# mezis/blurrily

Measured on AMD Instinct MI355X. Metric: find() queries/sec (batched), Geonames-scale haystack, higher is better.
Workload: dtype u32; 1 GPU; configs[2]: synthetic Geonames-scale haystack, 1M batched needles; haystack_strings=8423769, haystack_entries=117301316, needles_per_gpu=1000000, limit=10, index_replicated=False, parallelism=query-shard x1

## Files before the change

### blurrily_amd/csrc/find_kernels.h

```cpp
#pragma once
#include <hip/hip_runtime.h>

#include <cstddef>
#include <cstdint>

#include "../../include/blurrily_storage.h"
#include "device_index.h"

namespace blurrily {

struct TokeniseArgs {
  const char*     packed;
  const uint64_t* offsets;
  uint32_t        n;
  const uint32_t* code_total;
  uint16_t*       qcodes;
  uint32_t*       q_ntri;
  uint32_t*       q_nb;
  uint32_t*       big_list;
  uint32_t*       big_count;
  uint32_t*       mid_list;
  uint32_t*       mid_count;
  const uint32_t* start_win;
  uint32_t*       q_start;
  uint32_t        max_len;
};

struct FindArgs {
  const uint2*    slice_se;
  const uint16_t* ent;
  const uint32_t* ref_of_rank;
  const uint32_t* weight_of_rank;
  uint32_t        n_refs;
  uint32_t        n_windows;
  const uint64_t* offsets;
  const uint16_t* qcodes;
  const uint32_t* q_ntri;
  const uint32_t* q_nb;
  const uint32_t* q_start;
  const uint32_t* win_max_tri;
  uint32_t        nib_windows;
  const uint32_t* tomb;
  uint32_t        dense_min8;
  uint32_t        nm_dense;
  uint32_t        nm_cmin;
  uint32_t        own_only;
  uint32_t        cmin;
  const uint32_t* work_list;
  const uint32_t* n_work_dev;
  uint32_t        n_work;
  uint32_t*       queue;
  trigram_match_t* results;
  uint32_t*       counts;
  uint32_t        limit;
  uint32_t        keep;
  uint32_t        pass_base;
  uint32_t        pool_cap;
  unsigned long long* floor;
  uint32_t        short_only;
  uint32_t        ranges;
  unsigned long long* part_keys;
  uint32_t*       part_count;
  uint32_t*       over_list;
  uint32_t*       over_count;
  unsigned long long* phase_clocks;
  unsigned long long* stats;
  uint32_t*       path_flags;
};

enum : uint32_t {
  kPathNibble       = 1u << 0,
  kPathByte         = 1u << 1,
  kPathColdStart    = 1u << 2,
  kPathResweep      = 1u << 3,
  kPathCompaction   = 1u << 4,
  kPathSkipped      = 1u << 5,
  kPathRingOverflow = 1u << 6,
  kPathPipelined    = 1u << 7,
  kPathWide         = 1u << 8,
  kPathChunked      = 1u << 9,
  kPathRanged       = 1u << 10,
  kPathMultiPass    = 1u << 11,
  kPathTombstone    = 1u << 12,
  kPathOwnOnly      = 1u << 13,
  kPathWsTask       = 1u << 14,
  kPathWsLeftOut    = 1u << 15,
  kPathWsRobust     = 1u << 16,
  kPathWsCandOv     = 1u << 17,
  kPathWsPoolOv     = 1u << 18,
  kPathWsWide       = 1u << 19,
  kPathWsTableWalk  = 1u << 20,
  kPathNmLeftOut    = 1u << 21,
  kPathSmall        = 1u << 22,
};

enum : uint32_t {
  kStatPostingEntries = 0,
  kStatSteps          = 1,
  kStatTableWords     = 2,
  kStatTasks          = 3,
  kStatCompactions    = 4,
  kStatResweeps       = 5,
  kStatUnits          = 6,
  kStatProbes         = 7,
  kStatSlots          = 8,
  kStatWsClocks       = 8,
  kStatAllSlots       = 16,
};

void note_launch(const char* kernel_name);

uint32_t find_pool_cap(uint32_t keep);
bool find_can_leave(uint32_t keep);
int find_threads();
uint32_t find_wgs_per_cu();
int launch_tokenise(const TokeniseArgs& t, hipStream_t stream);
int launch_normalise(const char* in, const uint64_t* offsets, uint32_t n, char* out, uint32_t* non_ascii,
                     hipStream_t stream);
int launch_find(const FindArgs& a, bool long_needles, uint32_t grid, hipStream_t stream);
int launch_merge_parts(const FindArgs& a, uint32_t n_items, hipStream_t stream);
int launch_merge_parts_pinned(const FindArgs& a, uint32_t n_items, trigram_match_t* rows, uint32_t* words, uint32_t seq,
                              hipStream_t stream);
int launch_find_small(const FindArgs& a, uint32_t n_cus, hipStream_t stream);
constexpr uint32_t kSmallMaxKeep = 64, kSmallMaxWindows = 8;
constexpr uint32_t kOneMaxKeep = 120, kOneMaxGrid = 288, kOneMaxNeedles = 16, kMidMaxNeedles = 128;
int launch_find_one(const FindArgs& a, const uint16_t* codes, const uint32_t* T, uint32_t n_needles, uint32_t per, uint32_t grid,
                    unsigned long long* part_keys, uint32_t* flags, trigram_match_t* out_rows,
                    uint32_t* out_count, uint32_t seq, hipStream_t stream, uint32_t n_cus, const uint16_t* codes_far = nullptr,
                    const uint32_t* T_far = nullptr, uint32_t* tickets = nullptr);
int launch_wsweep(const FindArgs& a, uint32_t w, uint32_t n, uint32_t n_cus, bool own_pass, hipStream_t stream);
int launch_finalize_rows(const FindArgs& a, uint32_t n, hipStream_t stream);
constexpr uint32_t kWsMaxKeep = 128;

namespace counted {
int launch_find(const FindArgs& a, bool long_needles, uint32_t grid, hipStream_t stream);
int launch_find_small(const FindArgs& a, uint32_t n_cus, hipStream_t stream);
int launch_wsweep(const FindArgs& a, uint32_t w, uint32_t n, uint32_t n_cus, bool own_pass, hipStream_t stream);
int launch_finalize_rows(const FindArgs& a, uint32_t n, hipStream_t stream);
}
struct RefImage {
  const uint32_t* sorted_ref;
  const uint32_t* rank_of_pos;
  uint32_t        n_refs;
  const uint32_t* tomb;
  const uint2*    slice_se;
  const uint16_t* ent;
  const uint32_t* weight_of_rank;
  uint32_t        dense_min8;
  uint32_t        win0;
};
struct RefArgs {
  RefImage        img[2];
  uint32_t        n_img;
  uint32_t        n_win_all;
  const uint32_t* refs;
  uint32_t        n;
  uint2*          loc;
  uint32_t*       req;
  uint32_t*       win_cnt;
  uint64_t*       win_base;
  uint32_t*       wprefix;
  uint32_t*       slot_cnt;
  uint32_t*       slot_fill;
  uint64_t*       slot_start;
  uint16_t*       codes;
  uint32_t*       ntri;
  uint32_t*       weight;
  uint64_t*       qoff;
};
int launch_refs_extract(const RefArgs& a, hipStream_t stream);
struct RefNeedles {
  const uint16_t* codes;
  const uint64_t* qoff;
  const uint32_t* ntri;
  const uint32_t* weight;
  uint32_t        n;
  uint64_t        code_slots;
};
int launch_ref_needles(const RefNeedles& r, const uint32_t* code_total, const uint32_t* start_win, uint32_t* q_ntri,
                       uint32_t* q_nb, uint32_t* q_start, uint32_t* big_list, uint32_t* big_count, uint32_t* mid_list,
                       uint32_t* mid_count, hipStream_t stream);

struct ScopeMaskArgs {
  const uint2* loc;
  uint32_t     n;
  uint32_t     n_img;
  uint32_t     win0[2];
  uint32_t*    mask[2];
  uint32_t     mask_words[2];
};
int launch_scope_mask(const ScopeMaskArgs& a, hipStream_t stream);
constexpr uint32_t kScopeMaxKeep        = 256;
constexpr uint32_t kScopeMaxMembers     = 57344;
constexpr uint32_t kScopeMaxMemberCodes = 255;
struct ScopeFindArgs {
  const char*      packed;
  const uint64_t*  offsets;
  uint32_t         n;
  const uint32_t*  m_off;
  const uint16_t*  m_codes;
  const uint32_t*  m_ref;
  const uint32_t*  m_weight;
  uint32_t         n_members;
  uint32_t         limit;
  trigram_match_t* results;
  uint32_t*        counts;
};
int launch_scope_find(const ScopeFindArgs& a, hipStream_t stream);
struct ScopeDirect {
  const uint32_t* m_off;
  const uint16_t* m_codes;
  const uint32_t* m_ref;
  const uint32_t* m_weight;
  uint32_t        n_members;
  uint32_t        pad;
};
struct ScopeEachArgs {
  const char*        packed;
  const uint64_t*    offsets;
  const uint16_t*    codes;
  const uint64_t*    qoff;
  const uint32_t*    ntri;
  const uint2*       order;
  uint32_t           n;
  const ScopeDirect* scopes;
  uint32_t           max_members;
  uint32_t           limit;
  trigram_match_t*   results;
  uint32_t*          counts;
};
int launch_scope_each(const ScopeEachArgs& a, hipStream_t stream);
int launch_scope_gather_strings(const char* packed, const uint64_t* offsets, const uint32_t* idx, const uint64_t* out_off,
                                uint32_t n, char* out, hipStream_t stream);
int launch_scope_gather_refs(const RefNeedles& r, const uint32_t* idx, uint32_t n, uint64_t* qoff, uint32_t* ntri,
                             uint32_t* weight, hipStream_t stream);
int launch_scope_scatter(const trigram_match_t* rows, const uint32_t* counts, const uint32_t* idx, uint32_t n,
                         uint32_t limit, trigram_match_t* out_rows, uint32_t* out_counts, hipStream_t stream);

int launch_merge_rows(const trigram_match_t* a_rows, const uint32_t* a_counts, const trigram_match_t* b_rows,
                      const uint32_t* b_counts, uint32_t n, uint32_t limit, trigram_match_t* out,
                      uint32_t* out_counts, hipStream_t stream);

}
```

### blurrily_amd/csrc/kernels/needle_major.inc

```
constexpr uint32_t kRingUnitsMax = 512;
__host__ __device__ constexpr uint32_t ring_units_for(uint32_t pool_cap) {
  return pool_cap <= 512 ? kRingUnitsMax : 256u;
}
__device__ __forceinline__ uint32_t wave_inclusive_sum(uint32_t x) {
#define BLURRILY_DPP_ADD(ctrl_, rows_) x += uint32_t(__builtin_amdgcn_update_dpp(0, int(x), ctrl_, rows_, 0xF, false))
  BLURRILY_DPP_ADD(0x111, 0xF);
  BLURRILY_DPP_ADD(0x112, 0xF);
  BLURRILY_DPP_ADD(0x114, 0xF);
  BLURRILY_DPP_ADD(0x118, 0xF);
  BLURRILY_DPP_ADD(0x142, 0xA);
  BLURRILY_DPP_ADD(0x143, 0xC);
#undef BLURRILY_DPP_ADD
  return x;
}

struct UnitRing {
  uint4    hdr4[2];
  uint32_t hot[4][2][8];
};
constexpr uint32_t kNmMaxLeftOut = 8;
__device__ __forceinline__ uint32_t* pend_list(UnitRing* ring, uint32_t slot, uint32_t ring_units) {
  return reinterpret_cast<uint32_t*>(reinterpret_cast<uint2*>(ring + 1) + 2 * ring_units) + slot * kPendMax;
}

__device__ __forceinline__ bool coop_can_leave(const FindArgs& A) {
  return A.nm_cmin != 0 && A.pool_cap <= 1024 && !A.own_only && select_at(A) + 32 <= adm_max(A.pool_cap);
}

__device__ __forceinline__ void lds_barrier() { asm volatile("s_waitcnt lgkmcnt(0)\n\ts_barrier" ::: "memory"); }

enum : uint32_t { kLeftDone = 0, kLeftSlowScan = 2, kLeftSelect = 3 };

template <typename CT, int NT, bool MANAGER, bool LEARNS>
__device__ __forceinline__ void sweep_role(const FindArgs& A, const Needle& nd, const uint16_t* codes, uint32_t* cnt32,
                                           unsigned long long* pool, Control* ctl, UnitRing* ring, const uint8_t* wmt,
                                           const uint32_t w0, const uint32_t w1, const uint32_t ws) {
  constexpr bool kNib = std::is_same<CT, Nib>::value;
  constexpr uint32_t kWPS = kNib ? 2 : 1;
  constexpr uint32_t kNW = NT / 64, kWorkers = kNW - 1;
  const uint32_t tid = threadIdx.x;
  uint32_t lane;
  asm volatile("v_mbcnt_lo_u32_b32 %0, -1, 0\n\tv_mbcnt_hi_u32_b32 %0, -1, %0" : "=v"(lane));
  const uint32_t wid = MANAGER ? kWorkers : __builtin_amdgcn_readfirstlane(tid >> 6);
  const uint32_t tc = nd.T;
  const uint32_t v0 = w0 / kWPS, v1 = (w1 + kWPS - 1) / kWPS, vs = ws / kWPS;
  const uint32_t n_visit = v1 - v0;
  uint4* const cnt128 = reinterpret_cast<uint4*>(cnt32);
  const uint32_t ring_units = ring_units_for(A.pool_cap);
  const uint32_t sel_at = select_at(A);
  const bool can_leave = coop_can_leave(A);
  const uint32_t scan_pool_cap = can_leave ? A.pool_cap - adm_max(A.pool_cap) : A.pool_cap;
  const uint32_t pend_cap = can_leave ? min(kPendMax, adm_max(A.pool_cap) - sel_at) : 0u;
#define BLURRILY_STEP_AT(i_) ((i_) < n_visit ? (vs + (i_) < v1 ? vs + (i_) : vs + (i_) - n_visit) : v1)
#define BLURRILY_LOAD_WMT(base_)                                                 \
  do {                                                                           \
    const uint32_t i_ = (base_) + lane;                                          \
    uint32_t m_ = 0;                                                             \
    if (i_ < n_visit) {                                                          \
      const uint32_t p_ = BLURRILY_STEP_AT(i_) * kWPS;                           \
      if (wmt) {                      \
        m_ = wmt[p_];                                                            \
        if (kNib && p_ + 1 < w1) m_ = max(m_, uint32_t(wmt[p_ + 1]));            \
      } else {                                                                   \
        m_ = A.win_max_tri[p_];                                                  \
        if (kNib && p_ + 1 < w1) m_ = max(m_, A.win_max_tri[p_ + 1]);            \
      }                                                                          \
    }                                                                            \
    wm_l = m_; wm_base = (base_);                                                \
  } while (0)
#define BLURRILY_NEXT_VISIT(from_, out_)                                         \
  do {                                                                           \
    uint32_t f_ = (from_);                                                       \
    out_ = n_visit;                                                              \
    while (f_ < n_visit) {                                                       \
      const uint32_t b_ = f_ & ~63u;                                             \
      if (b_ != wm_base) BLURRILY_LOAD_WMT(b_);                                  \
      const uint32_t i_ = b_ + lane;                                             \
      const uint32_t need_l_ = matches_needed(thr_c, tc, BLURRILY_STEP_AT(i_) * kWPS * kWindowRanks); \
      const unsigned long long ok_ = __ballot(i_ < n_visit && min(tc, wm_l) >= need_l_) >> (f_ - b_); \
      if (ok_) { out_ = f_ + uint32_t(__builtin_ctzll(ok_)); break; }           \
      f_ = b_ + 64u;                                                             \
    }                                                                            \
  } while (0)
#define BLURRILY_FETCH_TABLE(p_, code_, A0, B0, A1, B1)                          \
  do {                                                                           \
    A0 = B0 = A1 = B1 = 0;                                                       \
    const uint32_t w_ = (p_) * kWPS;                                             \
    if (STATS(A) && w_ < w1) st_tab += 2u * tc * (kNib && w_ + 1 < w1 ? 2u : 1u); \
    if (w_ < w1 && lane < tc) {                                                  \
      const uint32_t idx_ = w_ * kNumCodes + (code_);                            \
      const uint2 se_ = A.slice_se[idx_]; A0 = se_.x; B0 = se_.y;                \
    }                                                                            \
    if (kNib && w_ + 1 < w1 && lane < tc) {                                      \
      const uint32_t idx_ = (w_ + 1) * kNumCodes + (code_);                      \
      const uint2 se_ = A.slice_se[idx_]; A1 = se_.x; B1 = se_.y;                \
    }                                                                            \
  } while (0)
#define BLURRILY_PUBLISH_HDR(s_, step_, nu_, need_, ls_)                         \
  do {                                                                           \
    const typename ScanTraits<CT>::Need nq_ = ScanTraits<CT>::prepare(need_);    \
    if (lane == 0) ring->hdr4[s_] = make_uint4((step_), (nu_) | ((need_) << 16) | ((ls_) << 24), nq_.bias, nq_.pre); \
  } while (0)
#define BLURRILY_TAB(s_) (reinterpret_cast<uint4*>(ring + 1) + (s_) * 64u)
#define BLURRILY_BND(s_) (reinterpret_cast<uint2*>(reinterpret_cast<uint4*>(ring + 1) + 128u) + (s_) * 64u)
#define BLURRILY_UNIT_OF(tb_, bd_, E_, k_, start_, end_, half_)                  \
  do {                                                                           \
    if (!kNib || (k_) < (E_)) {                                                  \
      const uint32_t t_ = uint32_t(__builtin_ctzll(__ballot((bd_).x > (k_)) | (1ull << 63))); \
      start_ = __builtin_amdgcn_readlane((tb_).x, t_) + ((k_) << 9);             \
      end_ = __builtin_amdgcn_readlane((tb_).z, t_);                             \
      half_ = 0u;                                                                \
    } else {                                                                     \
      const uint32_t t_ = uint32_t(__builtin_ctzll(__ballot((bd_).y > (k_)) | (1ull << 63))); \
      start_ = __builtin_amdgcn_readlane((tb_).y, t_) + ((k_) << 9);             \
      end_ = __builtin_amdgcn_readlane((tb_).w, t_);                             \
      half_ = 1u;                                                                \
    }                                                                            \
  } while (0)
#define BLURRILY_LEAVE_OUT(hs_, h_, A_, rk_, units_)                             \
  do {                                                                           \
    const bool skip_ = (rk_) < l_max_;                                           \
    const unsigned long long sm_ = __ballot(skip_);                              \
    if (skip_) {                                                                 \
      ring->hot[hs_][h_][__builtin_amdgcn_mbcnt_hi(uint32_t(sm_ >> 32), __builtin_amdgcn_mbcnt_lo(uint32_t(sm_), 0u))] = (A_); \
      units_ = 0;                                                                \
    }                                                                            \
    ls_ |= uint32_t(__popcll(sm_)) << (4u * (h_));                               \
  } while (0)
#define BLURRILY_RANK_ONE(A_, B_, rk_)                                           \
  do {                                                                           \
    const uint32_t size_ = (B_) - (A_);                                          \
    const bool dense_ = size_ >= A.nm_dense;                                     \
    uint32_t bigger_ = 0;                                                        \
    for (unsigned long long m_ = __ballot(dense_); m_; m_ &= m_ - 1) {           \
      const uint32_t u_ = __builtin_ctzll(m_);                                   \
      const uint32_t su_ = __builtin_amdgcn_readlane(size_, u_);                 \
      bigger_ += (su_ > size_ || (su_ == size_ && u_ < lane)) ? 1u : 0u;         \
    }                                                                            \
    rk_ = dense_ ? bigger_ : 0xFFu;                                              \
  } while (0)
#define BLURRILY_RANK()                                                          \
  do {                                                                           \
    BLURRILY_RANK_ONE(ta, tb, rk0);                                              \
    if (kNib) BLURRILY_RANK_ONE(ta1, tb1, rk1);                                  \
    ranked = true;                                                               \
  } while (0)
#define BLURRILY_PRODUCE(s_, hs_, step_, A0, B0, A1, B1)                         \
  do {                                                                           \
    const unsigned long long thr_ = thr_c;                                       \
    uint32_t need_ = min(matches_needed(thr_, tc, (step_) * kWPS * kWindowRanks), 0xFFu); \
    uint32_t units0_ = slice_units(A0, B0), units1_ = kNib ? slice_units(A1, B1) : 0u; \
    uint32_t ls_ = 0;                                                            \
             \
    const uint32_t l_max_ = (can_leave && thr_ != kKeyInf && need_ > A.nm_cmin) ? min(need_ - A.nm_cmin, kNmMaxLeftOut) : 0u; \
    if (l_max_) {                                                                \
      if (!ranked) BLURRILY_RANK();             \
      BLURRILY_LEAVE_OUT(hs_, 0u, A0, rk0, units0_);                             \
      if (kNib) BLURRILY_LEAVE_OUT(hs_, 1u, A1, rk1, units1_);                   \
    }                                                                            \
    ranked = false;                             \
    if (thr_ == kKeyInf && !nd.has_floor && !A.tomb && tc > 1) need_ = 0;        \
    const uint32_t incl0_ = wave_inclusive_sum(units0_);                         \
    const uint32_t even_ = __builtin_amdgcn_readlane(incl0_, 63);                \
    const uint32_t incl1_ = kNib ? even_ + wave_inclusive_sum(units1_) : even_;  \
    const uint32_t total_ = kNib ? __builtin_amdgcn_readlane(incl1_, 63) : even_; \
     \
    BLURRILY_TAB(s_)[lane] = make_uint4((A0) - ((incl0_ - units0_) << 9), (A1) - ((incl1_ - units1_) << 9), \
                                        units0_ ? (B0) : (A0) - ((incl0_ - units0_) << 9), units1_ ? (B1) : (A1) - ((incl1_ - units1_) << 9)); \
    BLURRILY_BND(s_)[lane] = make_uint2(incl0_, incl1_);                         \
     \
    const uint32_t lmost_ = max(ls_ & 15u, ls_ >> 4);                            \
    BLURRILY_PUBLISH_HDR(s_, step_, total_, need_ - min(need_, lmost_), ls_);    \
  } while (0)
#define BLURRILY_COUNT_UNITS(s_, n_, have_mine_)                                 \
  do {                                                                           \
    uint4 pend_ = make_uint4(0, 0, 0, 0);                                        \
    uint32_t pend_h_ = 0;                                                        \
    bool pend_live_ = false;                                                     \
    uint4 tl_ = tb_mine;                         \
    uint2 bl_ = bd_mine;                                                         \
    if (!(have_mine_)) { tl_ = BLURRILY_TAB(s_)[lane]; bl_ = BLURRILY_BND(s_)[lane]; } \
    const uint32_t even_ = kNib ? __builtin_amdgcn_readlane(bl_.x, 63) : 0u;     \
    uint32_t k_ = wid;                                                           \
    if ((have_mine_) && pre_valid) {             \
      pend_ = pre_v; pend_h_ = pre_h; pend_live_ = pre_live;                     \
      if (STATS(A) && wid < (n_)) {                                              \
        uint32_t x_, y_, h_;                                                     \
        BLURRILY_UNIT_OF(tl_, bl_, even_, wid, x_, y_, h_);                      \
        st_ent += min(512u, y_ - x_);                                            \
      }                                                                          \
      k_ = wid + kWorkers;                                                       \
    }                                                                            \
    pre_valid = false;                                                           \
    for (; k_ < (n_); k_ += kWorkers) {                                          \
      uint32_t x_, y_, h_;                                                       \
      BLURRILY_UNIT_OF(tl_, bl_, even_, k_, x_, y_, h_);                         \
      const bool live_ = lane8 < y_ - x_;                                        \
      uint4 v_ = pend_;                                                          \
      if (live_) v_ = *reinterpret_cast<const uint4*>(reinterpret_cast<const unsigned char*>(A.ent + x_) + lane16); \
      if (STATS(A)) st_ent += min(512u, y_ - x_);                                \
      if (pend_live_) bump_unit_loaded<CT>(cnt32, pend_, pend_h_);               \
      pend_ = v_; pend_h_ = h_; pend_live_ = live_;                              \
    }                                                                            \
    if (pend_live_) bump_unit_loaded<CT>(cnt32, pend_, pend_h_);                 \
  } while (0)
#define BLURRILY_PRELOAD()                                                       \
  do {                                                                           \
    const uint32_t np_ = __builtin_amdgcn_readfirstlane(h_next.x);               \
    const uint32_t nn_ = __builtin_amdgcn_readfirstlane(h_next.y) & 0xFFFFu;     \
    pre_valid = np_ < v1;                                                        \
    pre_live = false;                                                            \
    if (pre_valid && wid < nn_) {                                                \
      uint32_t x_, y_;                                                           \
      const uint32_t even_ = kNib ? __builtin_amdgcn_readlane(bd_mine.x, 63) : 0u; \
      BLURRILY_UNIT_OF(tb_mine, bd_mine, even_, wid, x_, y_, pre_h);             \
      pre_live = lane8 < y_ - x_;                                                \
      if (pre_live) pre_v = *reinterpret_cast<const uint4*>(reinterpret_cast<const unsigned char*>(A.ent + x_) + lane16); \
    }                                                                            \
  } while (0)
#define BLURRILY_COUNT_WALK(p_)                                                  \
  do {                                                                           \
    uint32_t fa0_, fb0_, fa1_, fb1_, k_ = 0;                                     \
    const uint32_t wcode_ = lane < tc ? codes[lane] : 0u;                        \
    BLURRILY_FETCH_TABLE(p_, wcode_, fa0_, fb0_, fa1_, fb1_);                    \
    BLURRILY_FOR_SLOT_UNITS(kNW, fa0_, fb0_, wid, lane, k_,                      \
                            { bump_unit<CT>(cnt32, load_group(A.ent, c, sb), 0u);   \
                              if (STATS(A)) st_ent += min(512u, sb - (c - lane * 8)); }); \
    if (kNib)                                                                    \
      BLURRILY_FOR_SLOT_UNITS(kNW, fa1_, fb1_, wid, lane, k_,                    \
                              { bump_unit<CT>(cnt32, load_group(A.ent, c, sb), 1u); \
                                if (STATS(A)) st_ent += min(512u, sb - (c - lane * 8)); }); \
  } while (0)
#define BLURRILY_MANAGER_TURN(e_, s_)                                            \
  do {                                                                           \
    if (my_i < n_visit) {                                                        \
      BLURRILY_PRODUCE((s_) ^ 1u, ((e_) + 1u) & 3u, BLURRILY_STEP_AT(my_i), ta, tb, ta1, tb1); \
    } else if (lane == 0) {                                                      \
      ring->hdr4[(s_) ^ 1u] = make_uint4(v1, 0u, 0u, 0u);                        \
    }                                                                            \
    PHASE_MARK(7);                                   \
    TRACE_MARK(A, nd.q, (e_), 1u, 7u);                                           \
    const uint32_t chosen_ = my_i;                                               \
    BLURRILY_NEXT_VISIT(chosen_ + 1, my_i);                                      \
    if (my_i != chosen_ + 1) PATH_FLAG(A, nd.q, kPathSkipped);                   \
    BLURRILY_FETCH_TABLE(BLURRILY_STEP_AT(my_i), mcode, ta, tb, ta1, tb1);       \
    PHASE_MARK(2);                                   \
  } while (0)
#define BLURRILY_PEND_SETTLE(slot_, hs_, pstep_, ls_)                            \
  do {                                                                           \
    const uint32_t np_ = min(uint32_t(__builtin_amdgcn_readfirstlane(ctl->pend_n[slot_])), pend_cap); \
    if (np_) {                                                                   \
      const uint32_t* const pl_ = pend_list(ring, slot_, ring_units);            \
      for (uint32_t c_ = lane; c_ < np_; c_ += 64) {                             \
        const uint32_t e_ = pl_[c_];                                             \
        const uint32_t h_ = (e_ >> 16) & 1u, r16_ = e_ & 0xFFFFu;                \
        const uint32_t L_ = ((ls_) >> (4u * h_)) & 15u;                          \
         \
        const uint4 ha_ = *reinterpret_cast<const uint4*>(&ring->hot[hs_][h_][0]); \
        const uint4 hb_ = *reinterpret_cast<const uint4*>(&ring->hot[hs_][h_][4]); \
        const uint32_t hs8_[kNmMaxLeftOut] = {ha_.x, ha_.y, ha_.z, ha_.w, hb_.x, hb_.y, hb_.z, hb_.w}; \
        uint32_t w_[kNmMaxLeftOut];                                              \
        _Pragma("unroll") for (uint32_t k_ = 0; k_ < kNmMaxLeftOut; ++k_) {      \
          w_[k_] = 0;                                                            \
          if (k_ < L_)                                                           \
            w_[k_] = reinterpret_cast<const uint32_t*>(A.ent + (hs8_[k_] - kBitmapSlots))[r16_ >> 5]; \
        }                                                                        \
        uint32_t cnt_ = e_ >> 20;                                                \
        _Pragma("unroll") for (uint32_t k_ = 0; k_ < kNmMaxLeftOut; ++k_) cnt_ += (w_[k_] >> (r16_ & 31u)) & 1u; \
        if (STATS(A)) atomicAdd(&STATS(A)[kStatProbes], static_cast<unsigned long long>(L_)); \
        const uint32_t rank_ = (pstep_) * kWPS * kWindowRanks + h_ * kWindowRanks + r16_; \
        const unsigned long long key_ = (static_cast<unsigned long long>(tc - min(tc, cnt_)) << 32) | rank_; \
        bool pass_ = key_ <= thr_c;                                              \
        if (nd.has_floor) pass_ = pass_ && key_ > ctl->floor;                    \
        if (pass_) {                                      \
          const uint32_t at_ = atomicAdd(&ctl->adm_n, 1u);                       \
          if (at_ < adm_max(A.pool_cap)) pool[A.pool_cap - adm_max(A.pool_cap) + at_] = key_; \
        }                                                                        \
      }                                                                          \
      if (lane == 0) ctl->pend_n[slot_] = 0;                                     \
    }                                                                            \
  } while (0)

  const uint32_t lane8 = lane * 8, lane16 = lane * 16;
  PHASE_DECL;
  uint32_t st_ent = 0, st_tab = 0, st_steps = 0, st_redo = 0;
  uint32_t mcode = 0, ta = 0, tb = 0, ta1 = 0, tb1 = 0, my_i = 0, p_prev = 0, ls_prev = 0;
  uint32_t rk0 = 0xFFu, rk1 = 0xFFu;
  bool ranked = false;
  uint32_t wm_l = 0, wm_base = 0xFFFFFFFFu;
  unsigned long long thr_c = ctl->thr;
  thr_c = (static_cast<unsigned long long>(__builtin_amdgcn_readfirstlane(uint32_t(thr_c >> 32))) << 32) |
          __builtin_amdgcn_readfirstlane(uint32_t(thr_c));
  uint4 tb_mine = make_uint4(0, 0, 0, 0);
  uint2 bd_mine = make_uint2(0, 0);
  uint4 pre_v = make_uint4(0, 0, 0, 0);
  uint32_t pre_h = 0;
  bool pre_live = false, pre_valid = false;
  (void)rk0; (void)rk1; (void)ranked; (void)wm_l; (void)wm_base; (void)thr_c; (void)mcode; (void)ta; (void)tb; (void)ta1; (void)tb1; (void)my_i; (void)p_prev; (void)ls_prev;
  (void)tb_mine; (void)bd_mine; (void)pre_v; (void)pre_h; (void)pre_live; (void)pre_valid; (void)lane8; (void)lane16; (void)pend_cap;
  if (MANAGER) PATH_FLAG(A, nd.q, kNib ? kPathNibble : kPathByte);
  if constexpr (MANAGER) {
    __builtin_amdgcn_s_setprio(3);
    mcode = lane < tc ? codes[lane] : 0u;
    BLURRILY_FETCH_TABLE(BLURRILY_STEP_AT(0u), mcode, ta, tb, ta1, tb1);
    BLURRILY_PRODUCE(0u, 0u, BLURRILY_STEP_AT(0u), ta, tb, ta1, tb1);
    BLURRILY_NEXT_VISIT(1u, my_i);
    BLURRILY_FETCH_TABLE(BLURRILY_STEP_AT(my_i), mcode, ta, tb, ta1, tb1);
  }
  bool have_thr = thr_c != kKeyInf;
  const uint32_t scan_cap = min(tc, ScanTraits<CT>::kMaxCount);
  __syncthreads();
  uint4 h_next = ring->hdr4[0];
  if constexpr (!MANAGER) { tb_mine = BLURRILY_TAB(0u)[lane]; bd_mine = BLURRILY_BND(0u)[lane]; }

  uint32_t e = 0;
  for (;;) {
    uint32_t left, s, p, n_units, hy_;
    for (;; ++e) {
      s = e & 1;
      p = __builtin_amdgcn_readfirstlane(h_next.x);
      hy_ = __builtin_amdgcn_readfirstlane(h_next.y);
      n_units = hy_ & 0xFFFFu;
      if (p >= v1) { left = kLeftDone; break; }
      ++st_steps;
      if constexpr (MANAGER) __builtin_amdgcn_s_setprio(3);
      PHASE_MARK(0);
      const bool tr_ = MANAGER || wid == 0;
      if (tr_) TRACE_MARK(A, nd.q, e, MANAGER ? 1u : 0u, 0u);
      if constexpr (MANAGER) {
        BLURRILY_MANAGER_TURN(e, s);
      } else {
        BLURRILY_COUNT_UNITS(s, n_units, true);
        PHASE_MARK(2);
      }
      if (tr_) TRACE_MARK(A, nd.q, e, MANAGER ? 1u : 0u, 1u);
      lds_barrier();
      if (tr_) TRACE_MARK(A, nd.q, e, MANAGER ? 1u : 0u, 2u);
      PHASE_MARK(3);
      const uint32_t nq_bias_ = __builtin_amdgcn_readfirstlane(h_next.z), nq_pre_ = __builtin_amdgcn_readfirstlane(h_next.w);
      h_next = ring->hdr4[s ^ 1u];
      if constexpr (!MANAGER) { tb_mine = BLURRILY_TAB(s ^ 1u)[lane]; bd_mine = BLURRILY_BND(s ^ 1u)[lane]; }
      if constexpr (MANAGER) {
        if (can_leave) {
          BLURRILY_PEND_SETTLE(s ^ 1u, (e - 1u) & 3u, p_prev, ls_prev);
          if (have_thr && n_units != 0 && ((hy_ >> 16) & 0xFFu) != 0) BLURRILY_RANK();
        }
        p_prev = p; ls_prev = n_units ? hy_ >> 24 : 0u;
      }
      if (n_units == 0) continue;
      const uint32_t need = (hy_ >> 16) & 0xFFu;
      if (need == 0) { left = kLeftSlowScan; break; }
      if constexpr (!MANAGER) {
        const uint32_t wbase = p * kWPS * kWindowRanks;
        const uint32_t wlen = min(kWPS * kWindowRanks, A.n_refs - wbase);
        typename ScanTraits<CT>::Need nq_ = ScanTraits<CT>::from_published(need, nq_bias_, nq_pre_);
        scan_core<CT, NT>(cnt128, nd, need, scan_cap, &ctl->thr, &ctl->floor, A.tomb, pool, scan_pool_cap, &ctl->pool_n,
                          &ctl->overflow, wbase, wlen, STATS(A) && A.path_flags ? &A.path_flags[nd.q] : nullptr,
                          hy_ >> 24, pend_list(ring, s, ring_units), &ctl->pend_n[s], pend_cap, uint32_t(NT - 64), &nq_);
        if (tr_) TRACE_MARK(A, nd.q, e, 0u, 3u);
        BLURRILY_PRELOAD();
      }
      if (tr_) TRACE_MARK(A, nd.q, e, MANAGER ? 1u : 0u, 4u);
      PHASE_MARK(5);
      lds_barrier();
      if (tr_) TRACE_MARK(A, nd.q, e, MANAGER ? 1u : 0u, 5u);
      PHASE_MARK(6);
      const uint4 c_ = *reinterpret_cast<const uint4*>(&ctl->pool_n);
      const uint32_t pn_ = c_.x + c_.z;
      const bool sel_ = (c_.y | uint32_t(pn_ > sel_at) | uint32_t(!have_thr && pn_ >= A.keep)) != 0;
      if (tr_) TRACE_MARK(A, nd.q, e, MANAGER ? 1u : 0u, 6u);
      if (__ballot(sel_) != 0) { left = kLeftSelect; break; }
    }
    const bool own_pending = can_leave && left == kLeftSelect && ctl->overflow == 0;
    if (can_leave) {
      if constexpr (MANAGER) {
        if (left == kLeftDone) BLURRILY_PEND_SETTLE((e & 1u) ^ 1u, (e - 1u) & 3u, p_prev, ls_prev);
        if (left == kLeftSelect && !own_pending && lane == 0) ctl->pend_n[s] = 0;
        p_prev = p; ls_prev = own_pending ? hy_ >> 24 : 0u;
        if (!ranked && have_thr && left != kLeftDone) BLURRILY_RANK();
      }
      __syncthreads();
    }
    if (left == kLeftDone) break;
    pre_valid = false;
    const uint32_t wbase = p * kWPS * kWindowRanks;
    const uint32_t wlen = min(kWPS * kWindowRanks, A.n_refs - wbase);
    bool scanned = left == kLeftSelect;
    for (;;) {
      if (!scanned) {
        scan_window<CT, NT, LEARNS>(A, nd, cnt128, pool, ctl, wbase, wlen, scan_pool_cap);
        __syncthreads();
      }
      scanned = false;
      if (!select_after_scan<NT>(A, pool, ctl, wbase, wlen, nd.q, scan_pool_cap)) break;
      ++st_redo;
      if ((hy_ >> 24) != 0) BLURRILY_COUNT_WALK(p);
      else if constexpr (!MANAGER) BLURRILY_COUNT_UNITS(s, n_units, false);
      __syncthreads();
    }
    thr_c = ctl->thr;
    thr_c = (static_cast<unsigned long long>(__builtin_amdgcn_readfirstlane(uint32_t(thr_c >> 32))) << 32) |
            __builtin_amdgcn_readfirstlane(uint32_t(thr_c));
    have_thr = thr_c != kKeyInf;
    ++e;
    h_next = ring->hdr4[e & 1];
    if constexpr (!MANAGER) { tb_mine = BLURRILY_TAB(e & 1)[lane]; bd_mine = BLURRILY_BND(e & 1)[lane]; }
  }
  if constexpr (MANAGER) PHASE_FLUSH_MANAGER(A); else PHASE_FLUSH(A);
  if (STATS(A) && A.path_flags && MANAGER && lane == 0) atomicAdd(&A.path_flags[nd.q], min(st_steps, 511u) << 23);
  if (STATS(A) && lane == 0) {
    atomicAdd(&STATS(A)[kStatPostingEntries], static_cast<unsigned long long>(st_ent));
    atomicAdd(&STATS(A)[kStatTableWords], static_cast<unsigned long long>(st_tab));
    if (wid == 0) {
      atomicAdd(&STATS(A)[kStatSteps], static_cast<unsigned long long>(st_steps));
      atomicAdd(&STATS(A)[kStatResweeps], static_cast<unsigned long long>(st_redo));
    }
  }
  if constexpr (MANAGER) __builtin_amdgcn_s_setprio(0);
  __syncthreads();
#undef BLURRILY_PEND_SETTLE
#undef BLURRILY_MANAGER_TURN
#undef BLURRILY_COUNT_WALK
#undef BLURRILY_COUNT_UNITS
#undef BLURRILY_PRELOAD
#undef BLURRILY_PRODUCE
#undef BLURRILY_RANK
#undef BLURRILY_RANK_ONE
#undef BLURRILY_LEAVE_OUT
#undef BLURRILY_UNIT_OF
#undef BLURRILY_TAB
#undef BLURRILY_PUBLISH_HDR
#undef BLURRILY_FETCH_TABLE
#undef BLURRILY_NEXT_VISIT
#undef BLURRILY_LOAD_WMT
#undef BLURRILY_STEP_AT
}

template <typename CT, int NT, bool LEARNS>
__device__ __forceinline__ void sweep_coop(const FindArgs& A, const Needle& nd, const uint16_t* codes, uint32_t* cnt32,
                                           unsigned long long* pool, Control* ctl, UnitRing* ring, const uint8_t* wmt,
                                           const uint32_t w0, const uint32_t w1, const uint32_t ws) {
  if (__builtin_amdgcn_readfirstlane(threadIdx.x >> 6) == NT / 64 - 1)
    sweep_role<CT, NT, true, LEARNS>(A, nd, codes, cnt32, pool, ctl, ring, wmt, w0, w1, ws);
  else
    sweep_role<CT, NT, false, LEARNS>(A, nd, codes, cnt32, pool, ctl, ring, wmt, w0, w1, ws);
}

template <typename CT, int NT, bool RANGED, bool SHORT>
__global__ __launch_bounds__(NT, (sizeof(CT) == 1 ? NT / 128 : NT / 256)) void find_kernel(const FindArgs A) {
  constexpr uint32_t kCntBytes = kWindowSize * sizeof(CT);
  __shared__ __attribute__((aligned(16))) uint32_t s_counters[kCntBytes / 4];
  extern __shared__ __attribute__((aligned(16))) unsigned char smem[];
  uint32_t* cnt32 = s_counters;
  uint4*    cnt128 = reinterpret_cast<uint4*>(s_counters);
  unsigned long long* pool = reinterpret_cast<unsigned long long*>(smem);
  uint32_t* s_tab = reinterpret_cast<uint32_t*>(pool + A.pool_cap);
  Control*  ctl = reinterpret_cast<Control*>(s_tab + 2 * kCodeChunk);
  UnitRing* ring = reinterpret_cast<UnitRing*>(reinterpret_cast<unsigned char*>(ctl) + 64);
  (void)ring;

  const uint32_t tid = threadIdx.x;

  for (uint32_t i = tid; i < kCntBytes / 16; i += NT) cnt128[i] = make_uint4(0, 0, 0, 0);
  const uint8_t* wmt = nullptr;
  if constexpr (SHORT) {
    if (A.n_windows <= 2 * kCodeChunk * 4) {
      uint8_t* w8 = reinterpret_cast<uint8_t*>(s_tab);
      for (uint32_t i = tid; i < A.n_windows; i += NT) w8[i] = uint8_t(min(A.win_max_tri[i], 255u));
      wmt = w8;
    }
  }
  (void)wmt;
  __syncthreads();

  const uint32_t n_work = A.n_work_dev ? *A.n_work_dev : A.n_work;

  PHASE_NEEDLE_DECL;
  for (;;) {
    __builtin_amdgcn_s_setprio(kSerialPrio);
    if (tid == 0) ctl->q = atomicAdd(A.queue, 1u);
    __syncthreads();
    const uint32_t slot = ctl->q;
    __syncthreads();
    if (slot >= n_work) break;
    const uint32_t R = RANGED ? A.ranges : 1u;
    const uint32_t n_items = RANGED ? n_work / R : 0u;
    const uint32_t item = RANGED ? slot % n_items : slot, range = RANGED ? R - 1u - slot / n_items : 0u;
    const uint32_t part = RANGED ? item * R + range : 0u;
    (void)part;
    const uint32_t q = A.work_list ? A.work_list[item] : item;
    const uint32_t n_pairs = (A.n_windows + 1) / 2;
    const bool own_only = !RANGED && A.own_only;
    const uint32_t own0 = own_only ? (A.q_start[q] & ~1u) : 0u;
    const uint32_t w0 = RANGED ? 2 * uint32_t(uint64_t(n_pairs) * range / R) : own0;
    const uint32_t w1 = RANGED ? min(A.n_windows, 2 * uint32_t(uint64_t(n_pairs) * (range + 1) / R))
                               : own_only ? min(A.n_windows, own0 + 2) : A.n_windows;
    Needle nd;
    nd.q = q;
    nd.T = A.q_ntri[q];
    nd.learn = false;
    if (!A.work_list && nd.T > (SHORT ? 64u : 127u)) {
      if (RANGED && tid == 0) A.part_count[part] = 0;
      if (RANGED) __syncthreads();
      continue;
    }
    const uint32_t have = A.pass_base ? A.counts[q] : 0u;
    if (A.q_nb[q] == 0 || A.keep == 0 || have < A.pass_base) {
      if (tid == 0 && A.pass_base == 0) {
        if (RANGED) A.part_count[part] = 0; else A.counts[q] = 0;
      }
      if (RANGED) __syncthreads();
      continue;
    }
    const uint16_t* codes = A.qcodes + A.offsets[q] + q;
    const uint32_t qs = A.q_start[q];
    const uint32_t ws = ((w1 - w0 >= 8 || own_only) && qs >= w0 && qs < w1) ? qs : w0;
    nd.has_floor = A.pass_base != 0;

    if (tid == 0) {
      ctl->pool_n = 0; ctl->overflow = 0; ctl->thr = kKeyInf;
      ctl->adm_n = 0; ctl->pend_n[0] = 0; ctl->pend_n[1] = 0;
      if (nd.has_floor) ctl->floor = A.floor[q];
    }
    __syncthreads();

    PHASE_NEEDLE(10);
    PATH_FLAG(A, q, (sizeof(CT) == 2 ? kPathWide : 0u) | (RANGED ? kPathRanged : 0u) | (nd.has_floor ? kPathMultiPass : 0u) |
                    (own_only ? kPathOwnOnly : 0u));
    __builtin_amdgcn_s_setprio(0);
    if (STATS(A) && tid == 0) atomicAdd(&STATS(A)[kStatTasks], 1ull);
#define BLURRILY_SWEEP(a_, b_, start_)                                                                  \
  do {                                                                                                  \
    const uint32_t sa = (a_), sb = (b_), st = (start_);                                                 \
    if constexpr (SHORT) {                                                                              \
            \
      const uint32_t nib_end = nd.T <= 15 ? sb : min(sb, max(sa, A.nib_windows));                       \
      if (nib_end < sb)                                                                                 \
        sweep_coop<CT, NT, RANGED>(A, nd, codes, cnt32, pool, ctl, ring, wmt, nib_end, sb, max(st, nib_end)); \
      if (sa < nib_end)                                                                                 \
        sweep_coop<Nib, NT, RANGED>(A, nd, codes, cnt32, pool, ctl, ring, wmt, sa, nib_end, min(st, nib_end - 1)); \
    } else if constexpr (sizeof(CT) == 1) {                \
      sweep_pipelined<CT, NT>(A, nd, codes, cnt32, pool, ctl, sa, sb, st);                              \
    } else {                                                                                            \
      if (nd.T <= kCodeChunk) sweep_pipelined<CT, NT>(A, nd, codes, cnt32, pool, ctl, sa, sb, st);    \
      else                    sweep_chunked<CT, NT>(A, nd, codes, cnt32, pool, s_tab, ctl, sa, sb);     \
    }                                                                                                   \
  } while (0)
    uint32_t sw_a = 0, sw_b = 0, sw_st = 0;
    (void)sw_a; (void)sw_b; (void)sw_st;
#define BLURRILY_SWEEP_ARGS(a_, b_, st_) do { sw_a = (a_); sw_b = (b_); sw_st = (st_); } while (0)
    if constexpr (RANGED) {
      const bool learn = qs < A.n_windows && !(qs >= w0 && qs < w1);
      for (uint32_t pass = learn ? 0u : 1u; pass < 2u; ++pass) {
        if (pass == 0) {
          BLURRILY_SWEEP_ARGS(qs, qs + 1, qs);
        } else {
          BLURRILY_SWEEP_ARGS(w0, w1, ws);
        }
        nd.learn = pass == 0;
        BLURRILY_SWEEP(sw_a, sw_b, sw_st);
        if (pass == 0) {
          compact_pool<NT>(pool, ctl, A.pool_cap, A.keep, SHORT && coop_can_leave(A) ? A.pool_cap - adm_max(A.pool_cap) : A.pool_cap);
          if (tid == 0) ctl->pool_n = 0;
          __syncthreads();
        }
      }
    } else {
      BLURRILY_SWEEP(w0, w1, ws);
    }
#undef BLURRILY_SWEEP_ARGS
#undef BLURRILY_SWEEP
    PHASE_NEEDLE(11);

    compact_pool<NT>(pool, ctl, A.pool_cap, A.keep, SHORT && coop_can_leave(A) ? A.pool_cap - adm_max(A.pool_cap) : A.pool_cap);
    __builtin_amdgcn_s_setprio(kSerialPrio);
    const uint32_t nres = ctl->pool_n;
    if (RANGED) {
      for (uint32_t i = tid; i < nres; i += NT) A.part_keys[size_t(part) * A.keep + i] = pool[i];
      if (tid == 0) A.part_count[part] = nres;
      __syncthreads();
      continue;
    }
    if (own_only) {
      uint32_t* st = reinterpret_cast<uint32_t*>(A.results + size_t(q) * A.limit);
      for (uint32_t i = tid; i < nres; i += NT) {
        const unsigned long long key = pool[i];
        st[2 * i] = uint32_t(key); st[2 * i + 1] = uint32_t(key >> 32);
      }
      if (tid == 0) A.counts[q] = nres;
      __syncthreads();
      continue;
    }
    trigram_match_t* out = A.results + size_t(q) * A.limit + A.pass_base;
    for (uint32_t i = tid; i < nres; i += NT) {
      const unsigned long long key = pool[i];
      const uint32_t rk = uint32_t(key);
      trigram_match_t r;
      r.reference = A.ref_of_rank[rk];
      r.matches = nd.T - uint32_t(key >> 32);
      r.weight = A.weight_of_rank[rk];
      out[i] = r;
    }
    if (tid == 0) {
      A.counts[q] = A.pass_base + nres;
      if (A.floor && nres > 0) A.floor[q] = pool[nres - 1];
    }
    __syncthreads();
    PHASE_NEEDLE(12);
  }
}
```

Measured before the change: 2.526 million queries/s.

## Precompute per-unit descriptors in manager so workers skip table unit lookup

The manager now scatters a per-unit (start,end) descriptor array for the first 64 units into LDS after the prefix sum, fills gaps with a DPP forward fill, and each worker lane preloads its own descriptor. Workers then read unit bounds via readlane instead of running the table/bound search (BLURRILY_UNIT_OF) per unit, falling back to the old path past 64 units. This aims to cut per-unit address computation in the hot counting loop, at the cost of extra LDS writes, wave barriers and DPP work on the manager. It also adds a stat counter for steps exceeding the descriptor range and makes n_work wave-uniform.

```diff
diff --git a/blurrily_amd/csrc/find_kernels.h b/blurrily_amd/csrc/find_kernels.h
--- a/blurrily_amd/csrc/find_kernels.h
+++ b/blurrily_amd/csrc/find_kernels.h
@@ -105,6 +105,7 @@
   kStatProbes         = 7,
   kStatSlots          = 8,
   kStatWsClocks       = 8,
+  kStatStepsPastDesc  = 14,
   kStatAllSlots       = 16,
 };
 
diff --git a/blurrily_amd/csrc/kernels/needle_major.inc b/blurrily_amd/csrc/kernels/needle_major.inc
--- a/blurrily_amd/csrc/kernels/needle_major.inc
+++ b/blurrily_amd/csrc/kernels/needle_major.inc
@@ -13,12 +13,33 @@
 #undef BLURRILY_DPP_ADD
   return x;
 }
+__device__ __forceinline__ void wave_fill_forward(uint2& d) {
+#define BLURRILY_DPP_FILL(ctrl_, rows_)                                                                        \
+  do {                                                                                                         \
+    const uint32_t px_ = uint32_t(__builtin_amdgcn_update_dpp(0, int(d.x), ctrl_, rows_, 0xF, false));         \
+    const uint32_t py_ = uint32_t(__builtin_amdgcn_update_dpp(0, int(d.y), ctrl_, rows_, 0xF, false));         \
+    const bool none_ = d.y == 0;                                                                               \
+    d.x = none_ ? px_ : d.x; d.y = none_ ? py_ : d.y;                                                          \
+  } while (0)
+  BLURRILY_DPP_FILL(0x111, 0xF);
+  BLURRILY_DPP_FILL(0x112, 0xF);
+  BLURRILY_DPP_FILL(0x114, 0xF);
+  BLURRILY_DPP_FILL(0x118, 0xF);
+  BLURRILY_DPP_FILL(0x142, 0xA);
+  BLURRILY_DPP_FILL(0x143, 0xC);
+#undef BLURRILY_DPP_FILL
+}
 
 struct UnitRing {
   uint4    hdr4[2];
   uint32_t hot[4][2][8];
 };
 constexpr uint32_t kNmMaxLeftOut = 8;
+constexpr uint32_t kDescUnits = 64;
+static_assert(kDescUnits == 64, "a lane of the manager per descriptor");
+constexpr uint32_t kRingTableBytes = 2 * 64 * 16 + 2 * 64 * 8 + 2 * kDescUnits * 8;
+static_assert(kRingTableBytes <= 2 * ring_units_for(512) * 8 && kRingTableBytes <= 2 * ring_units_for(1024) * 8,
+              "tables and descriptors lie in the ring area, in front of the pending lists (8 KiB and 4 KiB areas)");
 __device__ __forceinline__ uint32_t* pend_list(UnitRing* ring, uint32_t slot, uint32_t ring_units) {
   return reinterpret_cast<uint32_t*>(reinterpret_cast<uint2*>(ring + 1) + 2 * ring_units) + slot * kPendMax;
 }
@@ -28,6 +49,11 @@
 }
 
 __device__ __forceinline__ void lds_barrier() { asm volatile("s_waitcnt lgkmcnt(0)\n\ts_barrier" ::: "memory"); }
+__device__ __forceinline__ void wave_lds_sync() {
+  __builtin_amdgcn_fence(__ATOMIC_RELEASE, "wavefront");
+  __builtin_amdgcn_wave_barrier();
+  __builtin_amdgcn_fence(__ATOMIC_ACQUIRE, "wavefront");
+}
 
 enum : uint32_t { kLeftDone = 0, kLeftSlowScan = 2, kLeftSelect = 3 };
 
@@ -103,6 +129,14 @@
   } while (0)
 #define BLURRILY_TAB(s_) (reinterpret_cast<uint4*>(ring + 1) + (s_) * 64u)
 #define BLURRILY_BND(s_) (reinterpret_cast<uint2*>(reinterpret_cast<uint4*>(ring + 1) + 128u) + (s_) * 64u)
+#define BLURRILY_DESC(s_) (reinterpret_cast<uint2*>(reinterpret_cast<uint4*>(ring + 1) + 128u) + 128u + (s_) * kDescUnits)
+#define BLURRILY_DESC_MINE(s_) (BLURRILY_DESC(s_)[min(wid + kWorkers * lane, kDescUnits - 1u)])
+#define BLURRILY_UNIT_AT(ds_, j_, start_, end_, half_)                           \
+  do {                                                                           \
+    start_ = __builtin_amdgcn_readlane((ds_).x, (j_));                           \
+    end_ = __builtin_amdgcn_readlane((ds_).y, (j_));                             \
+    half_ = kNib ? (end_) & 1u : 0u;                                             \
+  } while (0)
 #define BLURRILY_UNIT_OF(tb_, bd_, E_, k_, start_, end_, half_)                  \
   do {                                                                           \
     if (!kNib || (k_) < (E_)) {                                                  \
@@ -164,43 +198,68 @@
     const uint32_t even_ = __builtin_amdgcn_readlane(incl0_, 63);                \
     const uint32_t incl1_ = kNib ? even_ + wave_inclusive_sum(units1_) : even_;  \
     const uint32_t total_ = kNib ? __builtin_amdgcn_readlane(incl1_, 63) : even_; \
+    const uint32_t ex0_ = incl0_ - units0_, ex1_ = incl1_ - units1_;              \
+    const uint32_t bs0_ = (A0) - (ex0_ << 9), bs1_ = (A1) - (ex1_ << 9);          \
      \
-    BLURRILY_TAB(s_)[lane] = make_uint4((A0) - ((incl0_ - units0_) << 9), (A1) - ((incl1_ - units1_) << 9), \
-                                        units0_ ? (B0) : (A0) - ((incl0_ - units0_) << 9), units1_ ? (B1) : (A1) - ((incl1_ - units1_) << 9)); \
+    uint2* const dsc_ = BLURRILY_DESC(s_);                                       \
+    dsc_[lane] = make_uint2(0u, 0u);                                             \
+    wave_lds_sync();                                                             \
+    if (units0_ && ex0_ < kDescUnits) dsc_[ex0_] = make_uint2(bs0_, (B0));       \
+    if (kNib && units1_ && ex1_ < kDescUnits) dsc_[ex1_] = make_uint2(bs1_, (B1) | 1u); \
+    wave_lds_sync();                             \
+    const unsigned long long dq_ = __hip_atomic_load(reinterpret_cast<unsigned long long*>(dsc_ + lane), __ATOMIC_RELAXED, \
+                                                     __HIP_MEMORY_SCOPE_WAVEFRONT); \
+    uint2 d_ = make_uint2(uint32_t(dq_), uint32_t(dq_ >> 32));                   \
+     \
+    BLURRILY_TAB(s_)[lane] = make_uint4(bs0_, bs1_, units0_ ? (B0) : bs0_, units1_ ? (B1) : bs1_); \
     BLURRILY_BND(s_)[lane] = make_uint2(incl0_, incl1_);                         \
+    wave_fill_forward(d_);                                                       \
+    dsc_[lane] = make_uint2(d_.x + (lane << 9), d_.y);    \
      \
     const uint32_t lmost_ = max(ls_ & 15u, ls_ >> 4);                            \
     BLURRILY_PUBLISH_HDR(s_, step_, total_, need_ - min(need_, lmost_), ls_);    \
   } while (0)
+#define BLURRILY_UNIT_STEP(x_, y_, h_)                                           \
+  do {                                                                           \
+    const bool live_ = lane8p < (y_) - (x_);     \
+    uint4 v_ = pend_;                                                            \
+    if (live_) v_ = *reinterpret_cast<const uint4*>(reinterpret_cast<const unsigned char*>(A.ent + (x_)) + lane16); \
+    if (STATS(A)) st_ent += min(512u, ((y_) & ~1u) - (x_));                      \
+    if (pend_live_) bump_unit_loaded<CT>(cnt32, pend_, pend_h_);                 \
+    pend_ = v_; pend_h_ = (h_); pend_live_ = live_;                              \
+  } while (0)
 #define BLURRILY_COUNT_UNITS(s_, n_, have_mine_)                                 \
   do {                                                                           \
     uint4 pend_ = make_uint4(0, 0, 0, 0);                                        \
     uint32_t pend_h_ = 0;                                                        \
     bool pend_live_ = false;                                                     \
-    uint4 tl_ = tb_mine;                         \
-    uint2 bl_ = bd_mine;                                                         \
-    if (!(have_mine_)) { tl_ = BLURRILY_TAB(s_)[lane]; bl_ = BLURRILY_BND(s_)[lane]; } \
-    const uint32_t even_ = kNib ? __builtin_amdgcn_readlane(bl_.x, 63) : 0u;     \
-    uint32_t k_ = wid;                                                           \
+    uint2 dl_ = ds_mine;                                                         \
+    if (!(have_mine_)) dl_ = BLURRILY_DESC_MINE(s_);                             \
+    uint32_t k_ = wid, j_ = 0;                                                   \
     if ((have_mine_) && pre_valid) {             \
       pend_ = pre_v; pend_h_ = pre_h; pend_live_ = pre_live;                     \
       if (STATS(A) && wid < (n_)) {                                              \
+        const uint32_t x_ = __builtin_amdgcn_readlane(dl_.x, 0), y_ = __builtin_amdgcn_readlane(dl_.y, 0); \
+        st_ent += min(512u, (y_ & ~1u) - x_);                                    \
+      }                                                                          \
+      k_ = wid + kWorkers; j_ = 1;                                               \
+    }                                                                            \
+    pre_valid = false;                                                           \
+    const uint32_t nd_ = min((n_), kDescUnits);                                  \
+    for (; k_ < nd_; k_ += kWorkers, ++j_) {                                     \
+      uint32_t x_, y_, h_;                                                       \
+      BLURRILY_UNIT_AT(dl_, j_, x_, y_, h_);                                     \
+      BLURRILY_UNIT_STEP(x_, y_, h_);                                            \
+    }                                                                            \
+    if ((n_) > kDescUnits) {                     \
+      const uint4 tl_ = BLURRILY_TAB(s_)[lane];                                  \
+      const uint2 bl_ = BLURRILY_BND(s_)[lane];                                  \
+      const uint32_t even_ = kNib ? __builtin_amdgcn_readlane(bl_.x, 63) : 0u;   \
+      for (; k_ < (n_); k_ += kWorkers) {                                        \
         uint32_t x_, y_, h_;                                                     \
-        BLURRILY_UNIT_OF(tl_, bl_, even_, wid, x_, y_, h_);                      \
-        st_ent += min(512u, y_ - x_);                                            \
+        BLURRILY_UNIT_OF(tl_, bl_, even_, k_, x_, y_, h_);                       \
+        BLURRILY_UNIT_STEP(x_, y_, h_);                                          \
       }                                                                          \
-      k_ = wid + kWorkers;                                                       \
-    }                                                                            \
-    pre_valid = false;                                                           \
-    for (; k_ < (n_); k_ += kWorkers) {                                          \
-      uint32_t x_, y_, h_;                                                       \
-      BLURRILY_UNIT_OF(tl_, bl_, even_, k_, x_, y_, h_);                         \
-      const bool live_ = lane8 < y_ - x_;                                        \
-      uint4 v_ = pend_;                                                          \
-      if (live_) v_ = *reinterpret_cast<const uint4*>(reinterpret_cast<const unsigned char*>(A.ent + x_) + lane16); \
-      if (STATS(A)) st_ent += min(512u, y_ - x_);                                \
-      if (pend_live_) bump_unit_loaded<CT>(cnt32, pend_, pend_h_);               \
-      pend_ = v_; pend_h_ = h_; pend_live_ = live_;                              \
     }                                                                            \
     if (pend_live_) bump_unit_loaded<CT>(cnt32, pend_, pend_h_);                 \
   } while (0)
@@ -212,9 +271,8 @@
     pre_live = false;                                                            \
     if (pre_valid && wid < nn_) {                                                \
       uint32_t x_, y_;                                                           \
-      const uint32_t even_ = kNib ? __builtin_amdgcn_readlane(bd_mine.x, 63) : 0u; \
-      BLURRILY_UNIT_OF(tb_mine, bd_mine, even_, wid, x_, y_, pre_h);             \
-      pre_live = lane8 < y_ - x_;                                                \
+      BLURRILY_UNIT_AT(ds_mine, 0u, x_, y_, pre_h);                              \
+      pre_live = lane8p < y_ - x_;                                               \
       if (pre_live) pre_v = *reinterpret_cast<const uint4*>(reinterpret_cast<const unsigned char*>(A.ent + x_) + lane16); \
     }                                                                            \
   } while (0)
@@ -281,9 +339,9 @@
     }                                                                            \
   } while (0)
 
-  const uint32_t lane8 = lane * 8, lane16 = lane * 16;
+  const uint32_t lane8p = lane * 8 + 1, lane16 = lane * 16;
   PHASE_DECL;
-  uint32_t st_ent = 0, st_tab = 0, st_steps = 0, st_redo = 0;
+  uint32_t st_ent = 0, st_tab = 0, st_steps = 0, st_redo = 0, st_past = 0;
   uint32_t mcode = 0, ta = 0, tb = 0, ta1 = 0, tb1 = 0, my_i = 0, p_prev = 0, ls_prev = 0;
   uint32_t rk0 = 0xFFu, rk1 = 0xFFu;
   bool ranked = false;
@@ -291,13 +349,12 @@
   unsigned long long thr_c = ctl->thr;
   thr_c = (static_cast<unsigned long long>(__builtin_amdgcn_readfirstlane(uint32_t(thr_c >> 32))) << 32) |
           __builtin_amdgcn_readfirstlane(uint32_t(thr_c));
-  uint4 tb_mine = make_uint4(0, 0, 0, 0);
-  uint2 bd_mine = make_uint2(0, 0);
+  uint2 ds_mine = make_uint2(0, 0);
   uint4 pre_v = make_uint4(0, 0, 0, 0);
   uint32_t pre_h = 0;
   bool pre_live = false, pre_valid = false;
   (void)rk0; (void)rk1; (void)ranked; (void)wm_l; (void)wm_base; (void)thr_c; (void)mcode; (void)ta; (void)tb; (void)ta1; (void)tb1; (void)my_i; (void)p_prev; (void)ls_prev;
-  (void)tb_mine; (void)bd_mine; (void)pre_v; (void)pre_h; (void)pre_live; (void)pre_valid; (void)lane8; (void)lane16; (void)pend_cap;
+  (void)ds_mine; (void)pre_v; (void)pre_h; (void)pre_live; (void)pre_valid; (void)lane8p; (void)lane16; (void)pend_cap;
   if (MANAGER) PATH_FLAG(A, nd.q, kNib ? kPathNibble : kPathByte);
   if constexpr (MANAGER) {
     __builtin_amdgcn_s_setprio(3);
@@ -311,7 +368,7 @@
   const uint32_t scan_cap = min(tc, ScanTraits<CT>::kMaxCount);
   __syncthreads();
   uint4 h_next = ring->hdr4[0];
-  if constexpr (!MANAGER) { tb_mine = BLURRILY_TAB(0u)[lane]; bd_mine = BLURRILY_BND(0u)[lane]; }
+  if constexpr (!MANAGER) ds_mine = BLURRILY_DESC_MINE(0u);
 
   uint32_t e = 0;
   for (;;) {
@@ -323,6 +380,7 @@
       n_units = hy_ & 0xFFFFu;
       if (p >= v1) { left = kLeftDone; break; }
       ++st_steps;
+      if (STATS(A) && n_units > kDescUnits) ++st_past;
       if constexpr (MANAGER) __builtin_amdgcn_s_setprio(3);
       PHASE_MARK(0);
       const bool tr_ = MANAGER || wid == 0;
@@ -339,7 +397,7 @@
       PHASE_MARK(3);
       const uint32_t nq_bias_ = __builtin_amdgcn_readfirstlane(h_next.z), nq_pre_ = __builtin_amdgcn_readfirstlane(h_next.w);
       h_next = ring->hdr4[s ^ 1u];
-      if constexpr (!MANAGER) { tb_mine = BLURRILY_TAB(s ^ 1u)[lane]; bd_mine = BLURRILY_BND(s ^ 1u)[lane]; }
+      if constexpr (!MANAGER) ds_mine = BLURRILY_DESC_MINE(s ^ 1u);
       if constexpr (MANAGER) {
         if (can_leave) {
           BLURRILY_PEND_SETTLE(s ^ 1u, (e - 1u) & 3u, p_prev, ls_prev);
@@ -404,7 +462,7 @@
     have_thr = thr_c != kKeyInf;
     ++e;
     h_next = ring->hdr4[e & 1];
-    if constexpr (!MANAGER) { tb_mine = BLURRILY_TAB(e & 1)[lane]; bd_mine = BLURRILY_BND(e & 1)[lane]; }
+    if constexpr (!MANAGER) ds_mine = BLURRILY_DESC_MINE(e & 1);
   }
   if constexpr (MANAGER) PHASE_FLUSH_MANAGER(A); else PHASE_FLUSH(A);
   if (STATS(A) && A.path_flags && MANAGER && lane == 0) atomicAdd(&A.path_flags[nd.q], min(st_steps, 511u) << 23);
@@ -414,6 +472,7 @@
     if (wid == 0) {
       atomicAdd(&STATS(A)[kStatSteps], static_cast<unsigned long long>(st_steps));
       atomicAdd(&STATS(A)[kStatResweeps], static_cast<unsigned long long>(st_redo));
+      atomicAdd(&STATS(A)[kStatStepsPastDesc], static_cast<unsigned long long>(st_past));
     }
   }
   if constexpr (MANAGER) __builtin_amdgcn_s_setprio(0);
@@ -422,12 +481,16 @@
 #undef BLURRILY_MANAGER_TURN
 #undef BLURRILY_COUNT_WALK
 #undef BLURRILY_COUNT_UNITS
+#undef BLURRILY_UNIT_STEP
 #undef BLURRILY_PRELOAD
 #undef BLURRILY_PRODUCE
 #undef BLURRILY_RANK
 #undef BLURRILY_RANK_ONE
 #undef BLURRILY_LEAVE_OUT
 #undef BLURRILY_UNIT_OF
+#undef BLURRILY_UNIT_AT
+#undef BLURRILY_DESC_MINE
+#undef BLURRILY_DESC
 #undef BLURRILY_TAB
 #undef BLURRILY_PUBLISH_HDR
 #undef BLURRILY_FETCH_TABLE
@@ -473,7 +536,7 @@
   (void)wmt;
   __syncthreads();
 
-  const uint32_t n_work = A.n_work_dev ? *A.n_work_dev : A.n_work;
+  const uint32_t n_work = __builtin_amdgcn_readfirstlane(A.n_work_dev ? *A.n_work_dev : A.n_work);
 
   PHASE_NEEDLE_DECL;
   for (;;) {
```

Result: faster. 2.607 million queries/s (median of 6 runs) (+3.2%).
